# imironhead/ml_super_resolution

Measured on AMD Instinct MI355X. Metric: VDSR-20 training patches/sec (41x41, batch 256 per GPU); fwd HR megapixels/sec alongside, higher is better.
Workload: dtype f32; 1 GPU; BASELINE configs[2]: VDSR 20-layer 3x3x64 residual, RGB, batch 256x41x41 per GPU, fwd+bwd+TF-Adam, random-init weights; global_batch=256, patch=41, parallelism=dp1

## Files before the change

### ml_super_resolution_amd/csrc/conv_narrow.hip

```cpp
#include "launchers.h"
namespace srx {
typedef float f32x3 __attribute__((ext_vector_type(3)));
typedef unsigned u32x3v __attribute__((ext_vector_type(3)));

template <int CTRL>
__device__ __forceinline__ float dpp_add(float v) {
    const int moved = __builtin_amdgcn_update_dpp(0, __float_as_int(v), CTRL, 0xf, 0xf, false);
    return v + __int_as_float(moved);
}

struct PixWalk {
    int n, oh, ow;
    __device__ __forceinline__ void init(unsigned p, int OH, int OW) {
        const unsigned t = p / (unsigned)OW;
        ow = (int)(p - t * (unsigned)OW);
        n = (int)(t / (unsigned)OH);
        oh = (int)(t - (unsigned)n * (unsigned)OH);
    }
    __device__ __forceinline__ void step16(int OH, int OW) { step(16, OH, OW); }
    __device__ __forceinline__ void step(int d, int OH, int OW) {
        ow += d;
        while (ow >= OW) {
            ow -= OW;
            oh += 1;
            if (oh == OH) { oh = 0; n += 1; }
        }
    }
};
template <int KH, int KW>
__device__ __forceinline__ void tap_offsets(int (&off)[KH * KW], const PixWalk& q, bool live, int H, int W, int pad_t, int pad_l,
                                            int PB, int lane_b) {
    const int centre = ((q.n * H + q.oh - pad_t) * W + (q.ow - pad_l)) * PB + lane_b;
    bool rok[KH], cok[KW];
#pragma unroll
    for (int kh = 0; kh < KH; ++kh) rok[kh] = live && (unsigned)(q.oh + kh - pad_t) < (unsigned)H;
#pragma unroll
    for (int kw = 0; kw < KW; ++kw) cok[kw] = (unsigned)(q.ow + kw - pad_l) < (unsigned)W;
#pragma unroll
    for (int kh = 0; kh < KH; ++kh)
#pragma unroll
        for (int kw = 0; kw < KW; ++kw)
            off[kh * KW + kw] = (rok[kh] && cok[kw]) ? centre + (kh * W + kw) * PB : kOobOffset;
}

template <int KH, int KW, int CIN, int CO>
__global__ __launch_bounds__(256) void conv_narrow_kernel(const ConvArgs a, long total_px, int iters) {
    static_assert(CIN == 64, "16 lanes x 4 channels per pixel");
    constexpr int TAPS = KH * KW;
    const int c4 = threadIdx.x & 15;
    const int sub = threadIdx.x >> 4;
    float wr[TAPS][4][CO];
#pragma unroll
    for (int t = 0; t < TAPS; ++t)
#pragma unroll
        for (int e = 0; e < 4; ++e)
#pragma unroll
            for (int c = 0; c < CO; ++c) wr[t][e][c] = a.w[((size_t)t * CIN + 4 * c4 + e) * CO + c];
    float bias[CO];
#pragma unroll
    for (int c = 0; c < CO; ++c) bias[c] = a.bias ? a.bias[c] : 0.0f;
    const __amdgpu_buffer_rsrc_t xrs = __builtin_amdgcn_make_buffer_rsrc(const_cast<float*>(a.x), 0,
                                                                         a.N * a.H * a.W * CIN * 4, 0x00020000);
    const unsigned p0 = blockIdx.x * (unsigned)iters * 16u + sub;
    PixWalk q;
    q.init(p0 < (unsigned)total_px ? p0 : 0u, a.OH, a.OW);
    for (int it = 0; it < iters; ++it, q.step16(a.OH, a.OW)) {
        const unsigned p = p0 + (unsigned)it * 16u;
        const bool live = p < (unsigned)total_px;
        int off[TAPS];
        tap_offsets<KH, KW>(off, q, live, a.H, a.W, a.pad_t, a.pad_l, CIN * 4, 16 * c4);
        f32x4 v[TAPS];
#pragma unroll
        for (int tp = 0; tp < TAPS; ++tp)
            v[tp] = __builtin_bit_cast(f32x4, __builtin_amdgcn_raw_buffer_load_b128(xrs, off[tp], 0, 0));
        float acc[CO];
#pragma unroll
        for (int c = 0; c < CO; ++c) acc[c] = 0.0f;
#pragma unroll
        for (int tp = 0; tp < TAPS; ++tp)
#pragma unroll
            for (int e = 0; e < 4; ++e)
#pragma unroll
                for (int c = 0; c < CO; ++c) acc[c] = fmaf(v[tp][e], wr[tp][e][c], acc[c]);
#pragma unroll
        for (int c = 0; c < CO; ++c) {
            float r = acc[c];
            r = dpp_add<0xB1>(r);
            r = dpp_add<0x4E>(r);
            r = dpp_add<0x124>(r);
            r = dpp_add<0x128>(r);
            acc[c] = r;
        }
        if (live && c4 < CO) {
            float r = (c4 == 0) ? acc[0] : (c4 == 1 ? acc[1 < CO ? 1 : 0] : acc[2 < CO ? 2 : 0]);
            r = act_apply(r + ((c4 == 0) ? bias[0] : (c4 == 1 ? bias[1 < CO ? 1 : 0] : bias[2 < CO ? 2 : 0])), a.act);
            const size_t o = (size_t)p * CO + c4;
            if (a.skip) r += a.skip[o];
            if (a.post_relu) r = act_apply(r, a.post_relu);
            a.y[o] = r;
        }
    }
}

template <int KH, int KW, bool NOUT, int CW = 64>
__global__ __launch_bounds__(256) void wgrad_narrow_kernel(const WgradArgs a, long total_px, int iters) {
    constexpr int TAPS = KH * KW, CN = 3;
    constexpr int LPP = CW / 4;
    constexpr int PPI = 256 / LPP;
    constexpr int NB = NOUT ? CN : 4;
    constexpr int NV = TAPS * 4 * CN + NB;
    __shared__ float red[4 * NV * LPP];
    const int c4 = threadIdx.x & (LPP - 1);
    const int sub = threadIdx.x / LPP;
    const int wave = threadIdx.x >> 6;
    float acc[NV];
#pragma unroll
    for (int i = 0; i < NV; ++i) acc[i] = 0.0f;
    const __amdgpu_buffer_rsrc_t xrs = __builtin_amdgcn_make_buffer_rsrc(
        const_cast<float*>(a.x), 0, a.N * a.H * a.W * (NOUT ? CW : CN) * 4, 0x00020000);
    const __amdgpu_buffer_rsrc_t drs = __builtin_amdgcn_make_buffer_rsrc(
        const_cast<float*>(a.dpre), 0, a.N * a.OH * a.OW * (NOUT ? CN : CW) * 4, 0x00020000);
    const unsigned p0 = blockIdx.x * (unsigned)iters * (unsigned)PPI + sub;
    PixWalk q;
    q.init(p0 < (unsigned)total_px ? p0 : 0u, a.OH, a.OW);
    for (int it = 0; it < iters; ++it, q.step(PPI, a.OH, a.OW)) {
        const unsigned p = p0 + (unsigned)it * (unsigned)PPI;
        const bool live = p < (unsigned)total_px;
        int off[TAPS];
        tap_offsets<KH, KW>(off, q, live, a.H, a.W, a.pad_t, a.pad_l, (NOUT ? CW : CN) * 4, NOUT ? 16 * c4 : 0);
        if constexpr (NOUT) {
            const f32x3 d = __builtin_bit_cast(f32x3, __builtin_amdgcn_raw_buffer_load_b96(drs, live ? (int)(p * CN * 4) : kOobOffset, 0, 0));
            f32x4 v[TAPS];
#pragma unroll
            for (int tp = 0; tp < TAPS; ++tp)
                v[tp] = __builtin_bit_cast(f32x4, __builtin_amdgcn_raw_buffer_load_b128(xrs, off[tp], 0, 0));
#pragma unroll
            for (int tp = 0; tp < TAPS; ++tp)
#pragma unroll
                for (int e = 0; e < 4; ++e)
#pragma unroll
                    for (int c = 0; c < CN; ++c) acc[(tp * 4 + e) * CN + c] = fmaf(v[tp][e], d[c], acc[(tp * 4 + e) * CN + c]);
#pragma unroll
            for (int c = 0; c < CN; ++c) acc[TAPS * 4 * CN + c] += d[c];
        } else {
            const f32x4 d = __builtin_bit_cast(f32x4, __builtin_amdgcn_raw_buffer_load_b128(
                drs, live ? (int)((p * CW + 4 * c4) * 4) : kOobOffset, 0, 0));
            f32x3 v[TAPS];
#pragma unroll
            for (int tp = 0; tp < TAPS; ++tp)
                v[tp] = __builtin_bit_cast(f32x3, __builtin_amdgcn_raw_buffer_load_b96(xrs, off[tp], 0, 0));
#pragma unroll
            for (int tp = 0; tp < TAPS; ++tp)
#pragma unroll
                for (int cn = 0; cn < CN; ++cn)
#pragma unroll
                    for (int e = 0; e < 4; ++e) acc[(tp * CN + cn) * 4 + e] = fmaf(v[tp][cn], d[e], acc[(tp * CN + cn) * 4 + e]);
#pragma unroll
            for (int e = 0; e < 4; ++e) acc[TAPS * 4 * CN + e] += d[e];
        }
    }
#pragma unroll
    for (int i = 0; i < NV; ++i) {
        float r = acc[i];
#pragma unroll
        for (int o = LPP; o < 64; o <<= 1) r += __shfl_xor(r, o);
        if (sub % (64 / LPP) == 0) red[(wave * NV + i) * LPP + c4] = r;
    }
    __syncthreads();
    float* part = a.part + (size_t)blockIdx.x * a.part_stride;
    const int wn = TAPS * CW * CN;
    for (int q = threadIdx.x; q < NV * LPP; q += 256) {
        const int i = q / LPP, l = q % LPP;
        const float r = (red[(0 * NV + i) * LPP + l] + red[(1 * NV + i) * LPP + l]) +
                        (red[(2 * NV + i) * LPP + l] + red[(3 * NV + i) * LPP + l]);
        if (i < TAPS * 4 * CN) {
            int idx;
            if constexpr (NOUT) {
                const int c = i % CN, te = i / CN, e = te & 3, tp = te >> 2;
                idx = (tp * CW + 4 * l + e) * CN + c;
            } else {
                const int e = i & 3, tc = i >> 2;
                idx = tc * CW + 4 * l + e;
            }
            part[idx] = r;
        } else {
            const int b = i - TAPS * 4 * CN;
            if constexpr (NOUT) {
                if (l == 0) part[wn + b] = r;
            } else {
                part[wn + 4 * l + b] = r;
            }
        }
    }
}

bool launch_wgrad_narrow(const ConvKey& k, const WgradArgs& a, int grid, hipStream_t s, hipError_t* err) {
    if (k.kh != 3 || k.kw != 3) return false;
    const bool nout = a.Cin == 64 && a.Cout == 3, nin = a.Cin == 3 && a.Cout == 64, nin32 = a.Cin == 3 && a.Cout == 32;
    if (!nout && !nin && !nin32) return false;
    const long total = (long)a.N * a.OH * a.OW;
    if (total >= (1L << 31) - 4096 || (long)a.N * a.H * a.W * 64 * 4 >= (1L << 31) - 4096 || total * 64 * 4 >= (1L << 31) - 4096)
        return false;
    const long ppi = nin32 ? 32 : 16;
    const int iters = (int)((total + ppi * grid - 1) / (ppi * grid));
    if (nout)
        hipLaunchKernelGGL((wgrad_narrow_kernel<3, 3, true>), dim3(grid), dim3(256), 0, s, a, total, iters);
    else if (nin)
        hipLaunchKernelGGL((wgrad_narrow_kernel<3, 3, false>), dim3(grid), dim3(256), 0, s, a, total, iters);
    else
        hipLaunchKernelGGL((wgrad_narrow_kernel<3, 3, false, 32>), dim3(grid), dim3(256), 0, s, a, total, iters);
    *err = hipGetLastError();
    return true;
}

bool launch_conv_narrow(const ConvKey& k, const ConvArgs& a, hipStream_t s, hipError_t* err) {
    if (k.wt || a.Cout != 3 || a.mask) return false;
    if ((long)a.N * a.H * a.W * a.Cin * 4 >= (1L << 31) - 4096) return false;
    const long total = (long)a.N * a.OH * a.OW;
    int iters = 16;
    while (iters > 1 && total / (16L * iters) < 2048) iters >>= 1;
    const long blocks = (total + 16L * iters - 1) / (16L * iters);
    if (total >= (1L << 31) - 4096) return false;
    if (k.kh == 3 && k.kw == 3 && a.Cin == 64) {
        hipLaunchKernelGGL((conv_narrow_kernel<3, 3, 64, 3>), dim3((unsigned)blocks), dim3(256), 0, s, a, total, iters);
    } else {
        return false;
    }
    *err = hipGetLastError();
    return true;
}
}
```

Before: 20210 patches/s.

## Use MFMA GEMM kernels for RGB-narrow conv forward and weight gradients

```diff
diff --git a/ml_super_resolution_amd/csrc/conv_narrow.hip b/ml_super_resolution_amd/csrc/conv_narrow.hip
--- a/ml_super_resolution_amd/csrc/conv_narrow.hip
+++ b/ml_super_resolution_amd/csrc/conv_narrow.hip
@@ -2,12 +2,6 @@
 namespace srx {
 typedef float f32x3 __attribute__((ext_vector_type(3)));
 typedef unsigned u32x3v __attribute__((ext_vector_type(3)));
-
-template <int CTRL>
-__device__ __forceinline__ float dpp_add(float v) {
-    const int moved = __builtin_amdgcn_update_dpp(0, __float_as_int(v), CTRL, 0xf, 0xf, false);
-    return v + __int_as_float(moved);
-}
 
 struct PixWalk {
     int n, oh, ow;
@@ -17,7 +11,6 @@
         n = (int)(t / (unsigned)OH);
         oh = (int)(t - (unsigned)n * (unsigned)OH);
     }
-    __device__ __forceinline__ void step16(int OH, int OW) { step(16, OH, OW); }
     __device__ __forceinline__ void step(int d, int OH, int OW) {
         ow += d;
         while (ow >= OW) {
@@ -43,66 +36,97 @@
             off[kh * KW + kw] = (rok[kh] && cok[kw]) ? centre + (kh * W + kw) * PB : kOobOffset;
 }
 
-template <int KH, int KW, int CIN, int CO>
-__global__ __launch_bounds__(256) void conv_narrow_kernel(const ConvArgs a, long total_px, int iters) {
-    static_assert(CIN == 64, "16 lanes x 4 channels per pixel");
-    constexpr int TAPS = KH * KW;
-    const int c4 = threadIdx.x & 15;
-    const int sub = threadIdx.x >> 4;
-    float wr[TAPS][4][CO];
-#pragma unroll
-    for (int t = 0; t < TAPS; ++t)
-#pragma unroll
-        for (int e = 0; e < 4; ++e)
-#pragma unroll
-            for (int c = 0; c < CO; ++c) wr[t][e][c] = a.w[((size_t)t * CIN + 4 * c4 + e) * CO + c];
-    float bias[CO];
-#pragma unroll
-    for (int c = 0; c < CO; ++c) bias[c] = a.bias ? a.bias[c] : 0.0f;
+constexpr int kOutZS = 29;
+constexpr int kOutTilePx = 560;
+struct OutTile {
+    int TH, TW, NTY, NTX;
+};
+__global__ __launch_bounds__(256, 2) void conv_rgb_out_kernel(const ConvArgs a, const OutTile g) {
+    constexpr int CIN = 64, CO = 3, NCOL = 27;
+    __shared__ float zs[kOutTilePx * kOutZS];
+    const int tid = threadIdx.x, lane = tid & 63, li = lane & 15, kq = lane >> 4;
+    const int wave = __builtin_amdgcn_readfirstlane(tid >> 6);
+    int t = blockIdx.x;
+    const int tx = t % g.NTX; t /= g.NTX;
+    const int ty = t % g.NTY, n = t / g.NTY;
+    const int oh0 = ty * g.TH, ow0 = tx * g.TW;
+    const int ZR = g.TH + 2, ZC = g.TW + 2, P = ZR * ZC;
+    float wr[2][16];
+#pragma unroll
+    for (int u = 0; u < 2; ++u) {
+        const int col = 16 * u + li;
+#pragma unroll
+        for (int s = 0; s < 16; ++s)
+            wr[u][s] = col < NCOL ? a.w[((col / CO) * CIN + 16 * (s >> 2) + 4 * kq + (s & 3)) * CO + col % CO] : 0.0f;
+    }
     const __amdgpu_buffer_rsrc_t xrs = __builtin_amdgcn_make_buffer_rsrc(const_cast<float*>(a.x), 0,
                                                                          a.N * a.H * a.W * CIN * 4, 0x00020000);
-    const unsigned p0 = blockIdx.x * (unsigned)iters * 16u + sub;
-    PixWalk q;
-    q.init(p0 < (unsigned)total_px ? p0 : 0u, a.OH, a.OW);
-    for (int it = 0; it < iters; ++it, q.step16(a.OH, a.OW)) {
-        const unsigned p = p0 + (unsigned)it * 16u;
-        const bool live = p < (unsigned)total_px;
-        int off[TAPS];
-        tap_offsets<KH, KW>(off, q, live, a.H, a.W, a.pad_t, a.pad_l, CIN * 4, 16 * c4);
-        f32x4 v[TAPS];
-#pragma unroll
-        for (int tp = 0; tp < TAPS; ++tp)
-            v[tp] = __builtin_bit_cast(f32x4, __builtin_amdgcn_raw_buffer_load_b128(xrs, off[tp], 0, 0));
-        float acc[CO];
-#pragma unroll
-        for (int c = 0; c < CO; ++c) acc[c] = 0.0f;
-#pragma unroll
-        for (int tp = 0; tp < TAPS; ++tp)
-#pragma unroll
-            for (int e = 0; e < 4; ++e)
-#pragma unroll
-                for (int c = 0; c < CO; ++c) acc[c] = fmaf(v[tp][e], wr[tp][e][c], acc[c]);
-#pragma unroll
-        for (int c = 0; c < CO; ++c) {
-            float r = acc[c];
-            r = dpp_add<0xB1>(r);
-            r = dpp_add<0x4E>(r);
-            r = dpp_add<0x124>(r);
-            r = dpp_add<0x128>(r);
-            acc[c] = r;
-        }
-        if (live && c4 < CO) {
-            float r = (c4 == 0) ? acc[0] : (c4 == 1 ? acc[1 < CO ? 1 : 0] : acc[2 < CO ? 2 : 0]);
-            r = act_apply(r + ((c4 == 0) ? bias[0] : (c4 == 1 ? bias[1 < CO ? 1 : 0] : bias[2 < CO ? 2 : 0])), a.act);
-            const size_t o = (size_t)p * CO + c4;
-            if (a.skip) r += a.skip[o];
-            if (a.post_relu) r = act_apply(r, a.post_relu);
-            a.y[o] = r;
-        }
-    }
-}
-
-template <int KH, int KW, bool NOUT, int CW = 64>
+    const auto pix_off = [&](int st) {
+        const int p = 16 * st + li, tr = p / ZC, tc = p - tr * ZC;
+        const int ih = oh0 - a.pad_t + tr, iw = ow0 - a.pad_l + tc;
+        const bool ok = p < P && (unsigned)ih < (unsigned)a.H && (unsigned)iw < (unsigned)a.W;
+        return ok ? ((n * a.H + ih) * a.W + iw) * (CIN * 4) + kq * 16 : kOobOffset;
+    };
+    const auto load4 = [&](f32x4 (&v)[4], int off) {
+#pragma unroll
+        for (int j = 0; j < 4; ++j) v[j] = __builtin_bit_cast(f32x4, __builtin_amdgcn_raw_buffer_load_b128(xrs, off, 64 * j, 0));
+    };
+    const int steps = (P + 15) >> 4;
+    const auto step = [&](const f32x4 (&cur)[4], f32x4 (&nxt)[4], int st) {
+        load4(nxt, pix_off(st + 4));
+        __builtin_amdgcn_sched_barrier(0);
+        f32x4 z0 = {0.f, 0.f, 0.f, 0.f}, z1 = {0.f, 0.f, 0.f, 0.f};
+#pragma unroll
+        for (int s = 0; s < 16; ++s) {
+            z0 = __builtin_amdgcn_mfma_f32_16x16x4f32(cur[s >> 2][s & 3], wr[0][s], z0, 0, 0, 0);
+            z1 = __builtin_amdgcn_mfma_f32_16x16x4f32(cur[s >> 2][s & 3], wr[1][s], z1, 0, 0, 0);
+        }
+        float* const zp = zs + (16 * st + 4 * kq) * kOutZS + li;
+#pragma unroll
+        for (int r = 0; r < 4; ++r) {
+            zp[r * kOutZS] = z0[r];
+            if (li < NCOL - 16) zp[r * kOutZS + 16] = z1[r];
+        }
+    };
+    constexpr int KV = (kOutTilePx * CO + 255) / 256;
+    const int th = a.OH - oh0 < g.TH ? a.OH - oh0 : g.TH, tw = a.OW - ow0 < g.TW ? a.OW - ow0 : g.TW;
+    const int nval = th * tw * CO;
+    int zo[KV];
+    unsigned yo[KV];
+    float sk[KV];
+#pragma unroll
+    for (int k = 0; k < KV; ++k) {
+        const int o = tid + 256 * k < nval ? tid + 256 * k : 0;
+        const int px = o / CO, c = o - px * CO, r = px / tw, cc = px - r * tw;
+        zo[k] = (r * ZC + cc) * kOutZS + c;
+        yo[k] = ((unsigned)(n * a.OH + oh0 + r) * (unsigned)a.OW + (unsigned)(ow0 + cc)) * CO + c;
+        sk[k] = (a.skip && tid + 256 * k < nval) ? a.skip[yo[k]] : 0.0f;
+    }
+    f32x4 va[4], vb[4];
+    load4(va, pix_off(wave));
+    for (int st = wave; st < steps; st += 8) {
+        step(va, vb, st);
+        if (st + 4 < steps) step(vb, va, st + 4);
+    }
+    __syncthreads();
+#pragma unroll
+    for (int k = 0; k < KV; ++k) {
+        if (tid + 256 * k < nval) {
+            const float* const z = zs + zo[k];
+            float t[9];
+#pragma unroll
+            for (int tap = 0; tap < 9; ++tap) t[tap] = z[((tap / 3) * ZC + tap % 3) * kOutZS + tap * CO];
+            const float sum = (((t[0] + t[1]) + (t[2] + t[3])) + ((t[4] + t[5]) + (t[6] + t[7]))) + t[8];
+            const int c = (tid + 256 * k) % CO;
+            float v = act_apply(sum + (a.bias ? a.bias[c] : 0.0f), a.act);
+            if (a.skip) v += sk[k];
+            if (a.post_relu) v = act_apply(v, a.post_relu);
+            a.y[yo[k]] = v;
+        }
+    }
+}
+
+template <int KH, int KW, bool NOUT, int CW>
 __global__ __launch_bounds__(256) void wgrad_narrow_kernel(const WgradArgs a, long total_px, int iters) {
     constexpr int TAPS = KH * KW, CN = 3;
     constexpr int LPP = CW / 4;
@@ -194,6 +218,168 @@
     }
 }
 
+constexpr int kRgbTilePx = 2048;
+constexpr int kRgbU = 8;
+template <bool NOUT>
+__global__ __launch_bounds__(256, 2) void wgrad_rgb_gemm_kernel(const WgradArgs a, int S, int Q, int qpw) {
+    constexpr int U = kRgbU, TAPS = 9, CN = 3, CW = 64;
+    __shared__ __attribute__((aligned(16))) float smem[kRgbTilePx * 4 + 4 * 2 * 64];
+    float* const bred = smem + kRgbTilePx * 4;
+    const int tid = threadIdx.x, lane = tid & 63, li = lane & 15, kq = lane >> 4;
+    const int wave = __builtin_amdgcn_readfirstlane(tid >> 6);
+    const int Hw = NOUT ? a.H : a.OH, Ww = NOUT ? a.W : a.OW;
+    const int Hn = NOUT ? a.OH : a.H, Wn = NOUT ? a.OW : a.W;
+    const int rlo = NOUT ? a.pad_t - 2 : -a.pad_t, clo = NOUT ? a.pad_l - 2 : -a.pad_l;
+    const int centre = a.pad_t * 3 + a.pad_l;
+    int jr[2], lcol[2];
+#pragma unroll
+    for (int u = 0; u < 2; ++u) {
+        const int n = 16 * u + li, tap = n < TAPS * CN ? n / CN : centre, c = n < TAPS * CN ? n % CN : 3;
+        const int kh = tap / 3, kw = tap % 3;
+        jr[u] = NOUT ? 2 - kh : kh;
+        lcol[u] = ((NOUT ? 2 - kw : kw) + kq) * 4 + c;
+    }
+    const __amdgpu_buffer_rsrc_t wrs = __builtin_amdgcn_make_buffer_rsrc(
+        const_cast<float*>(NOUT ? a.x : a.dpre), 0, a.N * Hw * Ww * CW * 4, 0x00020000);
+    const __amdgpu_buffer_rsrc_t nrs = __builtin_amdgcn_make_buffer_rsrc(
+        const_cast<float*>(NOUT ? a.dpre : a.x), 0, a.N * Hn * Wn * CN * 4, 0x00020000);
+    const int voff_full = kq * (CW * 4) + li * 16;
+    const int voff_last = (4 * (S - 1) + kq < Ww) ? voff_full : kOobOffset;
+    const int rowfix_g = (Ww - 4 * S) * (CW * 4);
+    const int PW = 4 * S + 2, rows_fit = kRgbTilePx / PW - 2, seg_quads = (kRgbTilePx / 3 - 2) / 4;
+
+    f32x4 acc[4][2];
+#pragma unroll
+    for (int t = 0; t < 4; ++t)
+#pragma unroll
+        for (int u = 0; u < 2; ++u) acc[t][u] = f32x4{0.f, 0.f, 0.f, 0.f};
+    [[maybe_unused]] float bsum[2] = {0.f, 0.f};
+
+    int q = blockIdx.x * qpw;
+    const int q1 = (Q - q < qpw) ? Q : q + qpw;
+    while (q < q1) {
+        const int r0 = q / S, s0 = q - r0 * S, n = r0 / Hw, h = r0 - n * Hw;
+        int qe, BR, tc0, PWb;
+        if (rows_fit >= 1) {
+            const int rows = rows_fit < Hw - h ? rows_fit : Hw - h;
+            qe = (r0 + rows) * S;
+            if (qe > q1) qe = q1;
+            BR = (qe - 1) / S - r0 + 1; tc0 = 0; PWb = PW;
+        } else {
+            int nq = S - s0 < seg_quads ? S - s0 : seg_quads;
+            if (nq > q1 - q) nq = q1 - q;
+            qe = q + nq; BR = 1; tc0 = 4 * s0; PWb = 4 * nq + 2;
+        }
+        __syncthreads();
+        for (int e = tid; e < (BR + 2) * PWb; e += 256) {
+            const int tr = e / PWb, tc = e - tr * PWb;
+            const int nr = h + rlo + tr, nc = tc0 + clo + tc;
+            const bool ok = (unsigned)nr < (unsigned)Hn && (unsigned)nc < (unsigned)Wn;
+            const f32x3 v = __builtin_bit_cast(f32x3, __builtin_amdgcn_raw_buffer_load_b96(
+                nrs, ok ? ((n * Hn + nr) * Wn + nc) * (CN * 4) : kOobOffset, 0, 0));
+            *reinterpret_cast<f32x4*>(smem + 4 * e) = f32x4{v[0], v[1], v[2], 1.0f};
+        }
+        __syncthreads();
+        const int per = (qe - q + 3) >> 2, wa = q + wave * per, wb = wa + per < qe ? wa + per : qe;
+        if (wa < wb) {
+            const int rw = wa / S, sw = wa - rw * S;
+            int ls = sw, lsoff = (rw * Ww + 4 * sw) * (CW * 4);
+            int cs = sw, coff = ((rw - r0) * PWb + 4 * sw - tc0) * 16;
+            const int rowfix_l = (PWb - 4 * S) * 16;
+            const int lb0 = (jr[0] * PWb * 4 + lcol[0]) * 4, lb1 = (jr[1] * PWb * 4 + lcol[1]) * 4;
+            const char* const tile = reinterpret_cast<const char*>(smem);
+            const auto load = [&](f32x4& v) {
+                v = __builtin_bit_cast(f32x4, __builtin_amdgcn_raw_buffer_load_b128(
+                                                  wrs, ls == S - 1 ? voff_last : voff_full, lsoff, 0));
+                ls += 1; lsoff += 4 * CW * 4;
+                lsoff += ls == S ? rowfix_g : 0;
+                ls = ls == S ? 0 : ls;
+            };
+            const auto mac = [&](const f32x4& v) {
+                const float b0 = *reinterpret_cast<const float*>(tile + (lb0 + coff));
+                const float b1 = *reinterpret_cast<const float*>(tile + (lb1 + coff));
+#pragma unroll
+                for (int t = 0; t < 4; ++t) {
+                    acc[t][0] = __builtin_amdgcn_mfma_f32_16x16x4f32(v[t], b0, acc[t][0], 0, 0, 0);
+                    acc[t][1] = __builtin_amdgcn_mfma_f32_16x16x4f32(v[t], b1, acc[t][1], 0, 0, 0);
+                }
+                if constexpr (NOUT) { bsum[0] += b0; bsum[1] += b1; }
+                cs += 1; coff += 4 * 16;
+                coff += cs == S ? rowfix_l : 0;
+                cs = cs == S ? 0 : cs;
+            };
+            f32x4 buf[U] = {};
+            const int total = wb - wa;
+            if (total >= U) {
+#pragma unroll
+                for (int j = 0; j < U; ++j) load(buf[j]);
+                int ahead = total - U;
+                for (; ahead >= U; ahead -= U) {
+#pragma unroll
+                    for (int j = 0; j < U; ++j) {
+                        mac(buf[j]);
+                        load(buf[j]);
+                        __builtin_amdgcn_sched_barrier(0);
+                    }
+                }
+#pragma unroll
+                for (int j = 0; j < U; ++j) {
+                    mac(buf[j]);
+                    if (j < ahead) load(buf[j]);
+                }
+#pragma unroll
+                for (int j = 0; j < U; ++j)
+                    if (j < ahead) mac(buf[j]);
+            } else {
+#pragma unroll
+                for (int j = 0; j < U; ++j)
+                    if (j < total) load(buf[j]);
+#pragma unroll
+                for (int j = 0; j < U; ++j)
+                    if (j < total) mac(buf[j]);
+            }
+        }
+        q = qe;
+    }
+    __syncthreads();
+#pragma unroll
+    for (int t = 0; t < 4; ++t)
+#pragma unroll
+        for (int u = 0; u < 2; ++u)
+#pragma unroll
+            for (int r = 0; r < 4; ++r) smem[(wave * 32 + (t * 2 + u) * 4 + r) * 64 + lane] = acc[t][u][r];
+    if constexpr (NOUT) {
+        bred[(wave * 2 + 0) * 64 + lane] = bsum[0];
+        bred[(wave * 2 + 1) * 64 + lane] = bsum[1];
+    }
+    __syncthreads();
+    float* const part = a.part + (size_t)blockIdx.x * a.part_stride;
+    constexpr int wn = TAPS * CW * CN;
+#pragma unroll
+    for (int m = 0; m < 8; ++m) {
+        const int idx = tid + 256 * m, reg = idx >> 6, l = idx & 63;
+        const float v = (smem[(0 * 32 + reg) * 64 + l] + smem[(1 * 32 + reg) * 64 + l]) +
+                        (smem[(2 * 32 + reg) * 64 + l] + smem[(3 * 32 + reg) * 64 + l]);
+        const int t = reg >> 3, u = (reg >> 2) & 1, r = reg & 3;
+        const int ch = 4 * (4 * (l >> 4) + r) + t, n = 16 * u + (l & 15);
+        if (n < TAPS * CN) {
+            if constexpr (NOUT) part[((n / CN) * CW + ch) * CN + n % CN] = v;
+            else part[n * CW + ch] = v;
+        } else if (!NOUT && n == TAPS * CN) {
+            part[wn + ch] = v;
+        }
+    }
+    if constexpr (NOUT) {
+        if (tid < CN) {
+            const int nc = centre * CN + tid, u = nc >> 4, j = nc & 15;
+            float v = 0.f;
+            for (int w = 0; w < 4; ++w)
+                for (int g = 0; g < 4; ++g) v += bred[(w * 2 + u) * 64 + g * 16 + j];
+            part[wn + tid] = v;
+        }
+    }
+}
+
 bool launch_wgrad_narrow(const ConvKey& k, const WgradArgs& a, int grid, hipStream_t s, hipError_t* err) {
     if (k.kh != 3 || k.kw != 3) return false;
     const bool nout = a.Cin == 64 && a.Cout == 3, nin = a.Cin == 3 && a.Cout == 64, nin32 = a.Cin == 3 && a.Cout == 32;
@@ -201,14 +387,20 @@
     const long total = (long)a.N * a.OH * a.OW;
     if (total >= (1L << 31) - 4096 || (long)a.N * a.H * a.W * 64 * 4 >= (1L << 31) - 4096 || total * 64 * 4 >= (1L << 31) - 4096)
         return false;
-    const long ppi = nin32 ? 32 : 16;
-    const int iters = (int)((total + ppi * grid - 1) / (ppi * grid));
-    if (nout)
-        hipLaunchKernelGGL((wgrad_narrow_kernel<3, 3, true>), dim3(grid), dim3(256), 0, s, a, total, iters);
-    else if (nin)
-        hipLaunchKernelGGL((wgrad_narrow_kernel<3, 3, false>), dim3(grid), dim3(256), 0, s, a, total, iters);
-    else
+    if (nin32) {
+        const long ppi = 32;
+        const int iters = (int)((total + ppi * grid - 1) / (ppi * grid));
         hipLaunchKernelGGL((wgrad_narrow_kernel<3, 3, false, 32>), dim3(grid), dim3(256), 0, s, a, total, iters);
+    } else {
+        if (a.pad_t > 1 || a.pad_l > 1) return false;
+        const int S = ((nout ? a.W : a.OW) + 3) / 4;
+        const long Q = (long)a.N * (nout ? a.H : a.OH) * S;
+        const int qpw = (int)((Q + grid - 1) / grid);
+        if (nout)
+            hipLaunchKernelGGL((wgrad_rgb_gemm_kernel<true>), dim3(grid), dim3(256), 0, s, a, S, (int)Q, qpw);
+        else
+            hipLaunchKernelGGL((wgrad_rgb_gemm_kernel<false>), dim3(grid), dim3(256), 0, s, a, S, (int)Q, qpw);
+    }
     *err = hipGetLastError();
     return true;
 }
@@ -217,15 +409,20 @@
     if (k.wt || a.Cout != 3 || a.mask) return false;
     if ((long)a.N * a.H * a.W * a.Cin * 4 >= (1L << 31) - 4096) return false;
     const long total = (long)a.N * a.OH * a.OW;
-    int iters = 16;
-    while (iters > 1 && total / (16L * iters) < 2048) iters >>= 1;
-    const long blocks = (total + 16L * iters - 1) / (16L * iters);
     if (total >= (1L << 31) - 4096) return false;
-    if (k.kh == 3 && k.kw == 3 && a.Cin == 64) {
-        hipLaunchKernelGGL((conv_narrow_kernel<3, 3, 64, 3>), dim3((unsigned)blocks), dim3(256), 0, s, a, total, iters);
-    } else {
-        return false;
-    }
+    if (k.kh != 3 || k.kw != 3 || a.Cin != 64 || a.pad_t > 1 || a.pad_l > 1) return false;
+    OutTile g;
+    const int strip = 30;
+    g.NTX = (kOutTilePx / (a.OW + 2) - 2 >= 4) ? 1 : (a.OW + strip - 1) / strip;
+    g.TW = (a.OW + g.NTX - 1) / g.NTX;
+    g.NTX = (a.OW + g.TW - 1) / g.TW;
+    const int th_max = kOutTilePx / (g.TW + 2) - 2;
+    g.NTY = (a.OH + th_max - 1) / th_max;
+    g.TH = (a.OH + g.NTY - 1) / g.NTY;
+    g.NTY = (a.OH + g.TH - 1) / g.TH;
+    const long blocks = (long)a.N * g.NTY * g.NTX;
+    if (blocks >= (1L << 31) - 4096) return false;
+    hipLaunchKernelGGL(conv_rgb_out_kernel, dim3((unsigned)blocks), dim3(256), 0, s, a, g);
     *err = hipGetLastError();
     return true;
 }
```

After: 20290 patches/s (median of 6 runs). No clear change (+0.4%).
